# ishine/TargetDiarization

Measured on AMD Instinct MI355X. Metric: real-time factor (audio-sec/wall-sec) full infer() pipe, 16kHz mono, 1/2/4/8 GPU, higher is better.
Workload: dtype f32 (split-f16 x3: fp32-accurate products from three f16 MFMA passes, fp32 accumulate); 1 GPU; BASELINE configs[3]: 1800 s synthetic conversation (two alternating speakers, 20 % overlap) = 180 x 10 s windows: MossFormer2 (90 windows per launch) -> loudness swap -> ERes2NetV2 on every 10 s window of both streams + cosine vs a target embedding -> Paraformer (SANM encoder, CIF predictor, NAR decoder, argmax tokens + timestamps) on 30 s segments of both streams -> CT-Transformer punctuation of ; windows_per_launch=90

## Files before the change

### targetdiarization_amd/csrc/gemm_h3.hpp

```cpp
#pragma once
#include <cstdio>
#include <cstdlib>
#include <typeinfo>
#include <vector>
#include <hip/hip_runtime.h>
#include <stdint.h>

#include "devutil.hpp"
#include "gemm.hpp"

namespace tdx {

typedef _Float16 f16x8 __attribute__((ext_vector_type(8)));

constexpr int H3_BM = 256, H3_BN = 256, H3_BK = 16, H3_THREADS = 512;
constexpr int H3_ROWB = 64;
constexpr int H3_OPER = 256 * H3_ROWB;
constexpr int H3_STAGE = 2 * H3_OPER;
constexpr int H3_NBUF = 4;
constexpr int H3_AUX_AHEAD = 3;
constexpr int H3_LDS = H3_NBUF * H3_STAGE;
constexpr int H3_LDS_EXTRA = 12288;

struct H3Seg {
// ... 725 lines not shown
                    __builtin_amdgcn_sched_barrier(0);
                    if (i + AH < 16) fetch(i + AH, (i + AH) % (AH + 1));
                    const int tn = i >> 3, tm = (i >> 1) & 3, half = i & 1;
                    RowT rw[8];
                    float sr[8];
                    int lb = lrow + tm * 32;
                    asm volatile("" : "+v"(lb));
#pragma unroll
                    for (int r8 = 0; r8 < 8; ++r8) {
                        const int r = half * 8 + r8;
                        const int lr = lb + (r & 3) + 8 * (r >> 2);
                        rw[r8] = row_of(lr);
                        sr[r8] = sal[lr];
                    }
#pragma unroll
                    for (int r8 = 0; r8 < 8; ++r8) touch(ax[i % (AH + 1)][r8]);
                    if (nn[tn] < g.N) {
#pragma unroll
                        for (int r8 = 0; r8 < 8; ++r8) {
                            const int r = half * 8 + r8;
                            const int lr = lb + (r & 3) + 8 * (r >> 2);
                            if constexpr (!CHECK && epi_has_full<Epi>::value) h3_assume_row(rw[r8]);
                            if (!CHECK || m0 + lr < g.M)
                                epi.store(z, m0 + lr, nn[tn], acc[tm][tn][r] * (sr[r8] * sc[tn]), rw[r8], cc[tn], ax[i % (AH + 1)][r8]);
                        }
                    }
                }
            } else {
#pragma unroll
                for (int tn = 0; tn < 2; ++tn) {
                    if (nn[tn] >= g.N) continue;
                    if constexpr (epi_has_ptr<Epi>::value) {
                        float* const p0 = epi.ptr(z, m0 + lrow, nn[tn]);
                        const long ldm = epi.ldm();
                        float sct = sc[tn];
                        if constexpr (epi_has_rowmul<Epi>::value) sct *= epi.colmul(cc[tn]);
#pragma unroll
                        for (int tm = 0; tm < 4; ++tm) {
#pragma unroll
                            for (int r = 0; r < 16; ++r) {
                                const int k = tm * 32 + (r & 3) + 8 * (r >> 2);
                                const RowT rw = row_of(lrow + k);
                                const float sr = sal[lrow + k];
                                if (!CHECK || m0 + lrow + k < g.M) {
                                    if constexpr (epi_has_rowmul<Epi>::value) epi.put_scaled(p0 + k * ldm, acc[tm][tn][r] * (sr * sct), rw, cc[tn]);
                                    else epi.put(p0 + k * ldm, acc[tm][tn][r] * (sr * sct), rw, cc[tn]);
                                }
                            }
                        }
                    } else {
#pragma unroll
                    for (int tm = 0; tm < 4; ++tm) {
#pragma unroll
                        for (int r = 0; r < 16; ++r) {
                            const int lr = lrow + tm * 32 + (r & 3) + 8 * (r >> 2);
                            const RowT rw = row_of(lr);
                            const float sr = sal[lr];
                            if constexpr (!CHECK && epi_has_full<Epi>::value) h3_assume_row(rw);
                            if (!CHECK || m0 + lr < g.M) epi.store(z, m0 + lr, nn[tn], acc[tm][tn][r] * (sr * sc[tn]), rw, cc[tn]);
                        }
                    }
                    }
                }
            }
        }
        }
    };

    auto epilogue_pl = [&](auto tag) {
        if constexpr (epi_has_plout<Epi>::value) {
        constexpr bool CHECK = decltype(tag)::value;
        int lrow = lrow0, lcol = lcol0;
        asm volatile("" : "+v"(lrow), "+v"(lcol));
        float* const T = reinterpret_cast<float*>(lds);
        const H3PlOut po = epi.plout(z);
        auto rowm = [&](int lr) { return CHECK ? min(m0 + lr, g.M - 1) : m0 + lr; };
        __syncthreads();
        if constexpr (PAIRED) {
            static_assert(epi_has_aux<Epi>::value && epi_has_pairmul<Epi>::value, "PLOUT PAIRED: gate-style functor");
            const int c = n0 + lcol;
            auto cc = epi.col(z, c);
            float sc0 = sb[(long)c * sbm], sc1 = sb[(long)(g.pair_off + c) * sbm];
            touch(cc); touch(sc0); touch(sc1);
            { const float2 pm = epi.pairmul(cc); sc0 *= pm.x; sc1 *= pm.y; }
            constexpr int AH = H3_AUX_AHEAD;
            decltype(epi.aux(0, 0, 0, RowT{})) ax[AH + 1][8];
            auto fetch = [&](int hb) {
                int lb = lrow + (hb >> 1) * 32;
                asm volatile("" : "+v"(lb));
#pragma unroll
                for (int r8 = 0; r8 < 8; ++r8) {
                    const int r = (hb & 1) * 8 + r8;
                    const int lr = lb + (r & 3) + 8 * (r >> 2);
                    ax[hb % (AH + 1)][r8] = epi.aux(z, rowm(lr), c, row_of(lr));
                }
            };
#pragma unroll
            for (int hb = 0; hb < AH; ++hb) fetch(hb);
#pragma unroll
            for (int hb = 0; hb < 8; ++hb) {
                __builtin_amdgcn_sched_barrier(0);
                if (hb + AH < 8) fetch(hb + AH);
                RowT rw[8];
                float sr[8];
                int lb = lrow + (hb >> 1) * 32;
                asm volatile("" : "+v"(lb));
#pragma unroll
                for (int r8 = 0; r8 < 8; ++r8) {
                    const int r = (hb & 1) * 8 + r8;
                    const int lr = lb + (r & 3) + 8 * (r >> 2);
                    rw[r8] = row_of(lr);
                    sr[r8] = sal[lr];
                }
#pragma unroll
                for (int r8 = 0; r8 < 8; ++r8) touch(ax[hb % (AH + 1)][r8]);
#pragma unroll
                for (int r8 = 0; r8 < 8; ++r8) {
                    const int tm = hb >> 1, r = (hb & 1) * 8 + r8;
                    const int lr = lb + (r & 3) + 8 * (r >> 2);
                    float v = epi.val2_scaled(z, m0 + lr, c, acc[tm][0][r] * (sr[r8] * sc0), acc[tm][1][r] * (sr[r8] * sc1), rw[r8], cc, ax[hb % (AH + 1)][r8]);
                    if (CHECK && m0 + lr >= g.M) v = 0.f;
                    T[lr * 128 + (lcol ^ (((lr >> 2) & 1) << 5))] = v;
                }
            }
            __syncthreads();
            H3_STAMP(3);
            const int hw = lane >> 5, l32 = lane & 31;
            unsigned char* const pbase = po.planes + (long)n0 * 4;
#pragma unroll 4
            for (int it = 0; it < 16; ++it) {
                const int rl = wave * 32 + it * 2 + hw;
                const int m = m0 + rl;
                const long pr = (!CHECK || m < g.M) ? epi.prow(z, min(m, g.M - 1)) : -1L;
                const f32x4 v4 = *reinterpret_cast<const f32x4*>(T + rl * 128 + ((4 * l32) ^ (((rl >> 2) & 1) << 5)));
                const float4 v = make_float4(v4[0], v4[1], v4[2], v4[3]);
                const float mu = h3_half_max(h3_absmax4(v));
                const float q2 = h3_half_sum((v.x * v.x + v.y * v.y) + (v.z * v.z + v.w * v.w));
                float inv;
                const float sc = h3_row_scale(mu, inv);
                h3_emit4_pred(pbase + (pr < 0 ? 0 : pr) * po.pitch, l32, v, sc, pr >= 0);
                if (l32 == 0 && pr >= 0) {
                    po.scale[(long)bn * po.seg_stride + pr] = inv;
                    if (po.ss) po.ss[(long)bn * po.seg_stride + pr] = q2;
                }
            }
        } else {
            int nn[2];
            decltype(epi.col(0, 0)) cc[2];
            float sc[2];
#pragma unroll
            for (int tn = 0; tn < 2; ++tn) {
                nn[tn] = n0 + tn * 128 + lcol;
                cc[tn] = epi.col(z, nn[tn]);
                sc[tn] = sb[(long)nn[tn] * sbm];
            }
            touch(cc[0]); touch(cc[1]); touch(sc[0]); touch(sc[1]);
            unsigned char* const pbase = po.planes + (long)n0 * 4;
            auto phase2 = [&](int hf) {
                __syncthreads();
#pragma unroll 4
                for (int it = 0; it < 16; ++it) {
                    const int rl = wave * 16 + it;
                    const int lr = (rl >> 6) * 128 + (2 * hf + ((rl >> 5) & 1)) * 32 + (rl & 31);
                    const int m = m0 + lr;
                    const long pr = (!CHECK || m < g.M) ? epi.prow(z, min(m, g.M - 1)) : -1L;
                    const f32x4 v4 = *reinterpret_cast<const f32x4*>(T + rl * 256 + ((4 * lane) ^ (((rl >> 2) & 1) << 5)));
                    const float4 v = make_float4(v4[0], v4[1], v4[2], v4[3]);
                    const float mu = h3_wave_max(h3_absmax4(v));
                    float q2 = (v.x * v.x + v.y * v.y) + (v.z * v.z + v.w * v.w);
                    if (po.ss) q2 = h3_wave_sum(q2);
                    float inv;
                    const float s_ = h3_row_scale(mu, inv);
                    if (pr >= 0) {
                        h3_emit4(pbase + pr * po.pitch, lane, v, s_);
                        if constexpr (epi_has_rowout<Epi>::value) *reinterpret_cast<f32x4*>(epi.rowout(z, pr, n0) + 4 * lane) = v4;
                        if (lane == 0) {
                            po.scale[(long)bn * po.seg_stride + pr] = inv;
                            if (po.ss) po.ss[(long)bn * po.seg_stride + pr] = q2;
                        }
                    }
                }
            };
            if constexpr (epi_has_aux<Epi>::value) {
                constexpr int AH = H3_AUX_AHEAD;
                decltype(epi.aux(0, 0, 0, RowT{})) ax[AH + 1][8];
                auto fetch = [&](int i, int set) {
                    const int tn = (i >> 2) & 1, tm = 2 * (i >> 3) + ((i >> 1) & 1), half = i & 1;
                    int lb = lrow + tm * 32;
                    asm volatile("" : "+v"(lb));
#pragma unroll
                    for (int r8 = 0; r8 < 8; ++r8) {
                        const int r = half * 8 + r8;
                        const int lr = lb + (r & 3) + 8 * (r >> 2);
                        ax[set][r8] = epi.aux(z, rowm(lr), nn[tn], row_of(lr));
                    }
                };
#pragma unroll
                for (int i = 0; i < AH; ++i) fetch(i, i % (AH + 1));
#pragma unroll
                for (int i = 0; i < 16; ++i) {
                    __builtin_amdgcn_sched_barrier(0);
                    if (i == 8) __syncthreads();
                    if (i + AH < 16) fetch(i + AH, (i + AH) % (AH + 1));
                    const int tn = (i >> 2) & 1, tmh = (i >> 1) & 1, tm = 2 * (i >> 3) + tmh, half = i & 1;
                    RowT rw[8];
                    float sr[8];
                    int lb = lrow + tm * 32;
                    asm volatile("" : "+v"(lb));
#pragma unroll
                    for (int r8 = 0; r8 < 8; ++r8) {
                        const int r = half * 8 + r8;
                        const int lr = lb + (r & 3) + 8 * (r >> 2);
                        rw[r8] = row_of(lr);
                        sr[r8] = sal[lr];
                    }
#pragma unroll
                    for (int r8 = 0; r8 < 8; ++r8) touch(ax[i % (AH + 1)][r8]);
#pragma unroll
                    for (int r8 = 0; r8 < 8; ++r8) {
                        const int r = half * 8 + r8;
                        const int lr = lb + (r & 3) + 8 * (r >> 2);
                        float v = 0.f;
                        if (!CHECK || m0 + lr < g.M) v = epi.val(z, m0 + lr, nn[tn], acc[tm][tn][r] * (sr[r8] * sc[tn]), rw[r8], cc[tn], ax[i % (AH + 1)][r8]);
                        const int rl = lr - wm * 64 - (tm - tmh) * 32;
                        T[rl * 256 + ((tn * 128 + lcol) ^ (((rl >> 2) & 1) << 5))] = v;
                    }
                    if (i == 7 || i == 15) phase2(i >> 3);
                }
            } else {
#pragma unroll
                for (int hf = 0; hf < 2; ++hf) {
                    if (hf) __syncthreads();
#pragma unroll
                    for (int tn = 0; tn < 2; ++tn) {
#pragma unroll
                        for (int tmh = 0; tmh < 2; ++tmh) {
                            const int tm = 2 * hf + tmh;
#pragma unroll
                            for (int r = 0; r < 16; ++r) {
                                const int lr = lrow + tm * 32 + (r & 3) + 8 * (r >> 2);
                                const RowT rw = row_of(lr);
                                const float sr = sal[lr];
                                float v = 0.f;
                                if (!CHECK || m0 + lr < g.M) v = epi.val(z, m0 + lr, nn[tn], acc[tm][tn][r] * (sr * sc[tn]), rw, cc[tn]);
                                const int rl = lr - wm * 64 - hf * 64 + 0 * tmh;
                                T[rl * 256 + ((tn * 128 + lcol) ^ (((rl >> 2) & 1) << 5))] = v;
                            }
                        }
                    }
                    phase2(hf);
                }
            }
        }
        }
    };

    auto epilogue_conv = [&]() {
        if constexpr (CONV) {
        int lrow = lrow0, lcol = lcol0;
        asm volatile("" : "+v"(lrow), "+v"(lcol));
        const H3Conv cv = epi.conv();
        int nn[2];
        decltype(epi.col(0, 0)) cc[2];
        float sc[2];
#pragma unroll
        for (int tn = 0; tn < 2; ++tn) {
            nn[tn] = n0 + tn * 128 + lcol;
            const int nc = min(nn[tn], g.N - 1);
            cc[tn] = epi.col(z, nc);
            sc[tn] = sb[(long)nc * sbm] * epi.colmul(cc[tn]);
        }
        touch(cc[0]); touch(cc[1]); touch(sc[0]); touch(sc[1]);
        if (n0 >= cv.ncols) {
#pragma unroll
            for (int tn = 0; tn < 2; ++tn) {
                if (nn[tn] >= g.N) continue;
                float* const p0 = epi.ptr(z, m0 + lrow, nn[tn]);
                const long ldm = epi.ldm();
#pragma unroll
                for (int tm = 0; tm < 4; ++tm) {
#pragma unroll
                    for (int r = 0; r < 16; ++r) {
                        const int k = tm * 32 + (r & 3) + 8 * (r >> 2);
                        const int lr = lrow + k;
                        const RowT rw = row_of(lr);
                        const float sr = sal[lr];
                        if (lr >= H3_CONV_HALO && lr < H3_CONV_HALO + H3_CONV_STEP && m0 + lr < g.M)
                            epi.put_scaled(p0 + k * ldm, acc[tm][tn][r] * (sr * sc[tn]), rw, cc[tn]);
                    }
                }
            }
            return;
        }
        float* const T = reinterpret_cast<float*>(lds);
        int* const sid = reinterpret_cast<int*>(lds + H3_LDS + 4096);
        const bool fast = m0 >= 0 && m0 + 255 < g.M && (m0 / cv.S) == ((m0 + 255) / cv.S);
        if (!fast && tid < 256) { const int m = m0 + tid; sid[tid] = (m >= 0 && m < g.M) ? m / cv.S : -1; }
        typedef float v2f __attribute__((ext_vector_type(2)));
        constexpr int KT = 17, HALF = 8, RW = 30;
        const int r_first = H3_CONV_HALO + RW * wave;
        __syncthreads();
        auto half = [&](auto tnc) {
            constexpr int tn = decltype(tnc)::value;
#pragma unroll
            for (int tm = 0; tm < 4; ++tm) {
#pragma unroll
                for (int j = 0; j < 4; ++j) {
                    const int lr = lrow + tm * 32 + 8 * j;
                    const f32x4 sr4 = *reinterpret_cast<const f32x4*>(sal + lr);
#pragma unroll
                    for (int i = 0; i < 4; ++i) T[(lr + i) * 128 + lcol] = (g.dbg & 16) ? acc[tm][tn][4 * j + i] : epi.act(acc[tm][tn][4 * j + i] * (sr4[i] * sc[tn]), cc[tn]);
                }
            }
            const int colp = n0 + tn * 128 + 2 * lane;
            v2f w[KT];
#pragma unroll
            for (int t = 0; t < KT; ++t) w[t] = *reinterpret_cast<const v2f*>(cv.w + (long)t * cv.wld + colp);
            __syncthreads();
            H3_STAMP(tn == 0 ? 3 : 6);
            const float* const Tc = T + 2 * lane;
            const unsigned poff = (unsigned)((colp >> 5) * 128 + (colp & 31) * 2);
            const bool has32 = cv.u32 && colp >= cv.u0;
            const unsigned uoff = (unsigned)(colp - cv.u0) * 4u;
            auto emit = [&](v2f o, long prow, long m) {
                typedef _Float16 h2 __attribute__((ext_vector_type(2)));
                const v2f xs = o * v2f{cv.sv, cv.sv};
                const h2 hi = h2{(_Float16)xs[0], (_Float16)xs[1]};
                const h2 lo = h2{(_Float16)(xs[0] - (float)hi[0]), (_Float16)(xs[1] - (float)hi[1])};
                unsigned char* const rowp = cv.planes + prow * cv.pitch;
                if (g.dbg & 4) { if (xs[0] == 123.456f) *reinterpret_cast<h2*>(rowp + poff) = lo; return; }
                *reinterpret_cast<h2*>(rowp + poff) = hi;
                *reinterpret_cast<h2*>(rowp + 64 + poff) = lo;
                if (has32) *reinterpret_cast<v2f*>(reinterpret_cast<unsigned char*>(cv.u32 + m * cv.ld32) + uoff) = o;
            };
            if (fast) {
                const int b0 = m0 / cv.S;
                const long prow0 = (long)b0 * cv.Sp + (m0 - b0 * cv.S);
                constexpr int RUN = 10;
#pragma unroll 1
                for (int r0 = r_first; r0 < r_first + RW; r0 += RUN) {
                    v2f win[RUN + KT - 1];
#pragma unroll
                    for (int i = 0; i < RUN + KT - 1; ++i) win[i] = *reinterpret_cast<const v2f*>(Tc + (r0 - HALF + i) * 128);
#pragma unroll
                    for (int i = 0; i < RUN; ++i) {
                        v2f o = win[HALF + i];
                        if (!(g.dbg & 8)) {
#pragma unroll
                            for (int t = 0; t < KT; ++t) o = __builtin_elementwise_fma(w[t], win[i + t], o);
                        }
                        emit(o, prow0 + r0 + i, (long)m0 + r0 + i);
                    }
                }
            } else {
#pragma unroll 1
                for (int lr = r_first; lr < r_first + RW; ++lr) {
                    const int so = sid[lr];
                    if (so < 0) continue;
                    v2f o = *reinterpret_cast<const v2f*>(Tc + lr * 128);
#pragma unroll
                    for (int t = 0; t < KT; ++t) {
                        const int rt = lr + t - HALF;
                        if (sid[rt] == so) o = __builtin_elementwise_fma(w[t], *reinterpret_cast<const v2f*>(Tc + rt * 128), o);
                    }
                    const long m = (long)m0 + lr;
                    emit(o, (long)so * cv.Sp + (m - (long)so * cv.S), m);
                }
            }
        };
        if (g.dbg & 32) return;
        half(std::integral_constant<int, 0>{});
        H3_STAMP(5);
        __syncthreads();
        half(std::integral_constant<int, 1>{});
        }
    };
    if constexpr (CONV) { epilogue_conv(); H3_STAMP(4); return; }
    bool whole = m0 + 256 <= g.M;
    if constexpr (epi_has_full<Epi>::value) whole = whole && epi.full(z, m0);
    if constexpr (epi_has_plout<Epi>::value) { if (whole) epilogue_pl(std::false_type{}); else epilogue_pl(std::true_type{}); }
    else { if (whole) epilogue(std::false_type{}); else epilogue(std::true_type{}); }
    H3_STAMP(4);
}

template <bool A_TR, bool B_TR, bool PAIRED, bool TWOSEG, class Epi, int VARIANT = 0, bool A_CONV = false>
inline hipError_t launch_gemm_h3x(H3Args g, int batches, Epi epi, hipStream_t st) {
    static const hipError_t attr_rc = hipFuncSetAttribute(reinterpret_cast<const void*>(&gemm_h3_kernel<A_TR, B_TR, PAIRED, TWOSEG, Epi, VARIANT, A_CONV>), hipFuncAttributeMaxDynamicSharedMemorySize,
                            H3_LDS + H3_LDS_EXTRA);
    (void)attr_rc;
    g.tiles_m = (g.M + H3_BM - 1) / H3_BM;
    if constexpr (epi_has_conv<Epi>::value) {
        g.tiles_m = (g.M + H3_CONV_STEP - 1) / H3_CONV_STEP;
        if (batches != 1 || g.seg[0].segk || g.seg[0].kchunk) return hipErrorInvalidValue;
    }
    g.tiles_n = PAIRED ? g.N / (H3_BN / 2) : (g.N + H3_BN - 1) / H3_BN;
    g.batches = batches;
    dim3 grid;
    if (g.tiles_m >= 16 && batches <= 4) {
        g.map_mode = 0;
        g.mp = (g.tiles_m + 7) / 8;
        long ktot = 0;
        for (int i = 0; i < g.nseg; ++i) ktot += g.seg[i].K;
        static const long gw_kb = [] { const char* e = getenv("TDX_H3_GW_KB"); return e ? atol(e) : 1536L; }();
        long gw = (gw_kb * 1024) / (256L * ktot * 4);
        if (gw < 1) gw = 1;
        if (gw > g.tiles_n) gw = g.tiles_n;
        g.gw = (int)gw;
        static const int mc_env = [] { const char* e = getenv("TDX_H3_MC"); return e ? atoi(e) : -1; }();
        g.mc = 0;
        if (g.gw < g.tiles_n) {
            long mc = mc_env >= 0 ? mc_env : (6L * 1024 * 1024) / (256L * ktot * 4);
            if (mc > 0 && mc < g.mp) g.mc = (int)mc;
        }
        grid = dim3(8 * g.mp * g.tiles_n, batches, 1);
    } else {
        g.map_mode = 1;
        g.mp = 0; g.gw = 1;
        grid = dim3(8 * ((batches + 7) / 8) * g.tiles_m * g.tiles_n, 1, 1);
    }
    if (TWOSEG && (g.seg[0].K < 64 || g.seg[1].K < 64 || g.seg[0].kchunk || g.seg[1].kchunk)) return hipErrorInvalidValue;
    for (int i = 0; i < g.nseg; ++i) {
        const H3Seg& sg = g.seg[i];
        if (sg.segk && (TWOSEG || A_TR || A_CONV || sg.segk % 64 || sg.K % sg.segk || sg.K / sg.segk > 8 || sg.kchunk)) return hipErrorInvalidValue;
        if ((sg.a_shift || sg.a_period) && (A_TR || A_CONV || (sg.a_period && !sg.a_zero))) return hipErrorInvalidValue;
    }
    if (epi_has_plout<Epi>::value && !PAIRED && g.N % 256) return hipErrorInvalidValue;
    if (A_CONV && (g.cv_cin < 64 || g.cv_cin % 16 || g.seg[0].K != g.cv_ntaps * g.cv_cin || !g.zero_row ||
                   batches != (g.cv_taps_total ? g.cv_taps_total / g.cv_ntaps : 1) || (g.cv_taps_total && g.cv_taps_total % g.cv_ntaps))) return hipErrorInvalidValue;
    static const int dbg = [] { const char* e = getenv("TDX_H3_DEBUG"); return e ? atoi(e) : 0; }();
    g.dbg = dbg;
#ifdef TDX_H3_STAMPS
    static int stamp_calls = 0;
    const long nblk = (long)grid.x * grid.y;
    if (!g.stamps && getenv("TDX_H3_STAMPS_DIR") && nblk >= 512 && ++stamp_calls == 4) {
        unsigned long long* buf = nullptr;
        hipMalloc((void**)&buf, nblk * 64);
        hipMemsetAsync(buf, 0, nblk * 64, st);
        g.stamps = buf;
        g.tiles_n = g.tiles_n;
        hipLaunchKernelGGL((gemm_h3_kernel<A_TR, B_TR, PAIRED, TWOSEG, Epi, VARIANT, A_CONV>), grid, dim3(H3_THREADS), H3_LDS + H3_LDS_EXTRA, st, g, epi);
        hipStreamSynchronize(st);
        std::vector<unsigned long long> hbuf(nblk * 8);
        hipMemcpy(hbuf.data(), buf, nblk * 64, hipMemcpyDeviceToHost);
        long ktot = 0;
        for (int i = 0; i < g.nseg; ++i) ktot += g.seg[i].K;
        char fn[512];
        snprintf(fn, sizeof fn, "%s/h3_%s_M%d_N%d_K%ld_z%d.bin", getenv("TDX_H3_STAMPS_DIR"), typeid(Epi).name(), g.M, g.N, ktot, batches);
        if (FILE* f = fopen(fn, "wb")) { fwrite(hbuf.data(), 8, hbuf.size(), f); fclose(f); }
        hipFree(buf);
        return hipGetLastError();
    }
#endif
    hipLaunchKernelGGL((gemm_h3_kernel<A_TR, B_TR, PAIRED, TWOSEG, Epi, VARIANT, A_CONV>), grid, dim3(H3_THREADS), H3_LDS + H3_LDS_EXTRA, st, g, epi);
    return hipGetLastError();
}

template <bool PAIRED, class Epi, int VARIANT = 0>
inline hipError_t launch_gemm_h3(H3Args g, int batches, Epi epi, hipStream_t st) {
    return launch_gemm_h3x<false, false, PAIRED, false, Epi, VARIANT>(g, batches, epi, st);
}


template <int UNUSED = 0>
__global__ __launch_bounds__(256) void h3_split_rows_kernel(const float* __restrict__ x, long ld, unsigned char* __restrict__ planes,
                                                           float* __restrict__ scale, long R, int K, int Kp) {
    const int lane = threadIdx.x & 63;
    const long row = (long)blockIdx.x * 4 + (threadIdx.x >> 6);
    if (row >= R) return;
    const float* xr = x + row * ld;
    float v[4][8];
    float mu = 0.f;
    const int nch = Kp / 8;
#pragma unroll
    for (int c = 0; c < 4; ++c) {
        const int ch = lane + 64 * c;
#pragma unroll
        for (int i = 0; i < 8; ++i) v[c][i] = 0.f;
        if (ch * 8 < K) {
            const f32x4 a = ldg4(xr + ch * 8), b = ldg4(xr + ch * 8 + 4);
#pragma unroll
            for (int i = 0; i < 4; ++i) { v[c][i] = a[i]; v[c][4 + i] = b[i]; }
        }
#pragma unroll
        for (int i = 0; i < 8; ++i) mu = fmaxf(mu, fabsf(v[c][i]));
    }
#pragma unroll
    for (int o = 32; o >= 1; o >>= 1) mu = fmaxf(mu, __shfl_xor(mu, o, 64));
    float inv;
    const float s = h3_row_scale(mu, inv);
    unsigned char* pr = planes + row * (long)Kp * 4;
#pragma unroll
    for (int c = 0; c < 4; ++c) {
        const int ch = lane + 64 * c;
        if (ch < nch) h3_store_chunk(pr + ch * 32, v[c], s);
    }
    if (lane == 0) scale[row] = inv;
}

template <int UNUSED = 0>
__global__ __launch_bounds__(256) void h3_split_rows_static_kernel(const float* __restrict__ x, long ld, unsigned char* __restrict__ planes,
                                                                  long R, int K, int Kp, float s) {
    const long i = (long)blockIdx.x * 256 + threadIdx.x;
    const int per = Kp / 8;
    if (i >= R * per) return;
    const long row = i / per;
    const int ch = (int)(i - row * per);
    float v[8];
#pragma unroll
    for (int j = 0; j < 8; ++j) v[j] = 0.f;
    if (ch * 8 < K) {
        const f32x4 a = ldg4(x + row * ld + ch * 8), b = ldg4(x + row * ld + ch * 8 + 4);
#pragma unroll
        for (int j = 0; j < 4; ++j) { v[j] = a[j]; v[4 + j] = b[j]; }
    }
    h3_store_chunk(planes + row * (long)Kp * 4 + ch * 32, v, s);
}
inline hipError_t launch_h3_split_rows_static(const float* x, long ld, void* planes, long R, int K, float s, hipStream_t st) {
    const int Kp = (K + 15) / 16 * 16;
    const long n = R * (Kp / 8);
    hipLaunchKernelGGL(h3_split_rows_static_kernel<0>, dim3((unsigned)((n + 255) / 256)), dim3(256), 0, st, x, ld, (unsigned char*)planes, R, K, Kp, s);
    return hipGetLastError();
}

template <int UNUSED = 0>
__global__ __launch_bounds__(256) void h3_split_rows_long_kernel(const float* __restrict__ x, long ld, unsigned char* __restrict__ planes,
                                                                float* __restrict__ scale, int K) {
    __shared__ float wmax[4];
    const long row = blockIdx.x;
    const float* xr = x + row * ld;
    float mu = 0.f;
    for (int k = threadIdx.x * 4; k < K; k += 1024) mu = fmaxf(mu, h3_absmax4(*reinterpret_cast<const float4*>(xr + k)));
    mu = h3_wave_max(mu);
    if ((threadIdx.x & 63) == 0) wmax[threadIdx.x >> 6] = mu;
    __syncthreads();
    mu = fmaxf(fmaxf(wmax[0], wmax[1]), fmaxf(wmax[2], wmax[3]));
    float inv;
    const float s = h3_row_scale(mu, inv);
    for (int ch = threadIdx.x; ch < K / 8; ch += 256) {
        const f32x4 a = ldg4(xr + ch * 8), b = ldg4(xr + ch * 8 + 4);
        const float v[8] = {a[0], a[1], a[2], a[3], b[0], b[1], b[2], b[3]};
        h3_store_chunk(planes + row * (long)K * 4 + ch * 32, v, s);
    }
    if (threadIdx.x == 0) scale[row] = inv;
}
inline hipError_t launch_h3_split_rows_long(const float* x, long ld, void* planes, float* scale, long R, int K, hipStream_t st) {
    hipLaunchKernelGGL(h3_split_rows_long_kernel<0>, dim3((unsigned)R), dim3(256), 0, st, x, ld, (unsigned char*)planes, scale, K);
    return hipGetLastError();
}

template <int UNUSED = 0>
__global__ __launch_bounds__(256) void h3_split_kmajor_kernel(const float* __restrict__ x, long ld, unsigned char* __restrict__ planes,
                                                             long K, int N, float s, const unsigned* __restrict__ mx,
                                                             float* __restrict__ inv, int S, int Sp) {
    const long i = (long)blockIdx.x * 256 + threadIdx.x;
    const int per = N / 8;
    if (i >= K * per) return;
    const long k = i / per;
    const int n = (int)(i - k * per) * 8;
    if (mx) {
        float iv;
        s = h3_row_scale(__uint_as_float(mx[0]), iv);
        if (i == 0) inv[0] = iv;
    }
    long src = k;
    bool ok = true;
    if (Sp > 0) { const long b = k / Sp; const int t = (int)(k - b * Sp); ok = t < S; src = b * S + t; }
    f32x4 a = {0.f, 0.f, 0.f, 0.f}, b4 = {0.f, 0.f, 0.f, 0.f};
    if (ok) { a = ldg4(x + src * ld + n); b4 = ldg4(x + src * ld + n + 4); }
    const float v[8] = {a[0], a[1], a[2], a[3], b4[0], b4[1], b4[2], b4[3]};
    f16x8 hi, lo;
#pragma unroll
    for (int j = 0; j < 8; ++j) {
        const float xs = v[j] * s;
        const _Float16 t = (_Float16)xs;
        hi[j] = t; lo[j] = (_Float16)(xs - (float)t);
    }
    unsigned char* dst = planes + k * (4L * N) + (n >> 5) * 128 + ((n & 31) >> 3) * 16;
    *reinterpret_cast<f16x8*>(dst) = hi;
    *reinterpret_cast<f16x8*>(dst + 64) = lo;
}

template <int UNUSED = 0>
__global__ __launch_bounds__(256) void h3_absmax_kernel(const float* __restrict__ x, long n, unsigned* __restrict__ mx) {
    float m = 0.f;
    for (long i = (long)blockIdx.x * 256 + threadIdx.x; i < n; i += (long)gridDim.x * 256) m = fmaxf(m, fabsf(x[i]));
    m = h3_wave_max(m);
    if ((threadIdx.x & 63) == 0) atomicMax(mx, __float_as_uint(m));
}

inline hipError_t launch_h3_split_rows(const float* x, long ld, void* planes, float* scale, long R, int K, hipStream_t st) {
    const int Kp = (K + 15) / 16 * 16;
    hipLaunchKernelGGL(h3_split_rows_kernel<0>, dim3((unsigned)((R + 3) / 4)), dim3(256), 0, st, x, ld, (unsigned char*)planes, scale, R, K, Kp);
    return hipGetLastError();
}

}
```

Baseline: 512.0 audio-s/s.

## Widen conv epilogue stores via lane permutes and swizzled LDS staging

Reworks the fused depthwise-conv epilogue of the split-f16 GEMM. Each lane now owns a column permutation, and staged tiles in LDS use an XOR-swizzled column layout. Two adjacent output rows are exchanged across lanes with permlane32/permlane16 swaps, so hi/lo f16 plane writes and fp32 side-output writes become 16-byte stores instead of scattered 4/8-byte stores. The FMA loop is reordered tap-outer to expose independent accumulators. In exchange it adds permute instructions and register pressure, and it depends on the has32 region starting at the tile column base, a coarser check than the previous per-column one.

After: 514.9 audio-s/s, median of 6. Within noise of the previous version (+0.6%).

```diff
diff --git a/targetdiarization_amd/csrc/gemm_h3.hpp b/targetdiarization_amd/csrc/gemm_h3.hpp
--- a/targetdiarization_amd/csrc/gemm_h3.hpp
+++ b/targetdiarization_amd/csrc/gemm_h3.hpp
@@ -1051,54 +1051,81 @@
         __syncthreads();
         auto half = [&](auto tnc) {
             constexpr int tn = decltype(tnc)::value;
-#pragma unroll
-            for (int tm = 0; tm < 4; ++tm) {
-#pragma unroll
-                for (int j = 0; j < 4; ++j) {
-                    const int lr = lrow + tm * 32 + 8 * j;
-                    const f32x4 sr4 = *reinterpret_cast<const f32x4*>(sal + lr);
-#pragma unroll
-                    for (int i = 0; i < 4; ++i) T[(lr + i) * 128 + lcol] = (g.dbg & 16) ? acc[tm][tn][4 * j + i] : epi.act(acc[tm][tn][4 * j + i] * (sr4[i] * sc[tn]), cc[tn]);
-                }
-            }
-            const int colp = n0 + tn * 128 + 2 * lane;
+            const int pcol = 32 * ((lcol >> 1) & 3) + ((((lcol >> 2) & ~1) | (lcol & 1)) ^ (8 * ((lcol >> 1) & 3)));
+            auto stage = [&](auto actc) {
+#pragma unroll
+                for (int tm = 0; tm < 4; ++tm) {
+#pragma unroll
+                    for (int j = 0; j < 4; ++j) {
+                        const int lr = lrow + tm * 32 + 8 * j;
+                        const f32x4 sr4 = *reinterpret_cast<const f32x4*>(sal + lr);
+#pragma unroll
+                        for (int i = 0; i < 4; ++i)
+                            T[(lr + i) * 128 + pcol] = decltype(actc)::value ? epi.act(acc[tm][tn][4 * j + i] * (sr4[i] * sc[tn]), cc[tn]) : acc[tm][tn][4 * j + i];
+                    }
+                }
+            };
+            if (g.dbg & 16) stage(std::false_type{});
+            else stage(std::true_type{});
+            const int colbase = n0 + tn * 128;
+            const int colp = colbase + 8 * (lane & 15) + 2 * (lane >> 4);
             v2f w[KT];
 #pragma unroll
             for (int t = 0; t < KT; ++t) w[t] = *reinterpret_cast<const v2f*>(cv.w + (long)t * cv.wld + colp);
             __syncthreads();
             H3_STAMP(tn == 0 ? 3 : 6);
-            const float* const Tc = T + 2 * lane;
-            const unsigned poff = (unsigned)((colp >> 5) * 128 + (colp & 31) * 2);
-            const bool has32 = cv.u32 && colp >= cv.u0;
-            const unsigned uoff = (unsigned)(colp - cv.u0) * 4u;
-            auto emit = [&](v2f o, long prow, long m) {
-                typedef _Float16 h2 __attribute__((ext_vector_type(2)));
+            const float* const Tc = T + 32 * (lane >> 4) + ((2 * (lane & 15)) ^ (8 * (lane >> 4)));
+            const bool has32 = cv.u32 && colbase >= cv.u0;
+            typedef _Float16 h2 __attribute__((ext_vector_type(2)));
+            auto split = [&](v2f o, unsigned& hiw, unsigned& low) {
                 const v2f xs = o * v2f{cv.sv, cv.sv};
                 const h2 hi = h2{(_Float16)xs[0], (_Float16)xs[1]};
                 const h2 lo = h2{(_Float16)(xs[0] - (float)hi[0]), (_Float16)(xs[1] - (float)hi[1])};
-                unsigned char* const rowp = cv.planes + prow * cv.pitch;
-                if (g.dbg & 4) { if (xs[0] == 123.456f) *reinterpret_cast<h2*>(rowp + poff) = lo; return; }
-                *reinterpret_cast<h2*>(rowp + poff) = hi;
-                *reinterpret_cast<h2*>(rowp + 64 + poff) = lo;
-                if (has32) *reinterpret_cast<v2f*>(reinterpret_cast<unsigned char*>(cv.u32 + m * cv.ld32) + uoff) = o;
+                hiw = __builtin_bit_cast(unsigned, hi); low = __builtin_bit_cast(unsigned, lo);
             };
             if (fast) {
                 const int b0 = m0 / cv.S;
                 const long prow0 = (long)b0 * cv.Sp + (m0 - b0 * cv.S);
+                const int t4 = lane >> 4, b16 = lane & 15;
+                const unsigned pofs = (unsigned)(colbase * 4 + (b16 >> 2) * 128 + (t4 & 1) * 64 + (b16 & 3) * 16 + (t4 >> 1) * cv.pitch);
+                const unsigned uofs = (unsigned)(((colbase - cv.u0) + 8 * b16 + 4 * (t4 & 1)) * 4 + (t4 >> 1) * cv.ld32 * 4);
+                auto swap32 = [](unsigned& x, unsigned& y) { const auto r = __builtin_amdgcn_permlane32_swap(x, y, false, false); x = r[0]; y = r[1]; };
+                auto swap16 = [](unsigned& x, unsigned& y) { const auto r = __builtin_amdgcn_permlane16_swap(x, y, false, false); x = r[0]; y = r[1]; };
                 constexpr int RUN = 10;
 #pragma unroll 1
                 for (int r0 = r_first; r0 < r_first + RW; r0 += RUN) {
                     v2f win[RUN + KT - 1];
 #pragma unroll
                     for (int i = 0; i < RUN + KT - 1; ++i) win[i] = *reinterpret_cast<const v2f*>(Tc + (r0 - HALF + i) * 128);
-#pragma unroll
-                    for (int i = 0; i < RUN; ++i) {
-                        v2f o = win[HALF + i];
-                        if (!(g.dbg & 8)) {
-#pragma unroll
-                            for (int t = 0; t < KT; ++t) o = __builtin_elementwise_fma(w[t], win[i + t], o);
+                    v2f o[RUN];
+#pragma unroll
+                    for (int i = 0; i < RUN; ++i) o[i] = win[HALF + i];
+                    if (!(g.dbg & 8)) {
+#pragma unroll
+                        for (int t = 0; t < KT; ++t)
+#pragma unroll
+                            for (int i = 0; i < RUN; ++i) o[i] = __builtin_elementwise_fma(w[t], win[i + t], o[i]);
+                    }
+                    unsigned char* const rowp = cv.planes + (prow0 + r0) * cv.pitch;
+                    unsigned char* const urow = reinterpret_cast<unsigned char*>(cv.u32 + ((long)m0 + r0) * cv.ld32);
+                    if (g.dbg & 4) {
+                        if (o[0][0] == 123.456f && o[RUN - 1][1] == 123.456f) *reinterpret_cast<v2f*>(rowp) = o[0];
+                        continue;
+                    }
+#pragma unroll
+                    for (int p = 0; p < RUN; p += 2) {
+                        unsigned x0, x1, x2, x3;
+                        split(o[p], x0, x1); split(o[p + 1], x2, x3);
+                        swap32(x0, x2); swap32(x1, x3); swap16(x0, x1); swap16(x2, x3);
+                        *reinterpret_cast<uint4*>(rowp + (long)p * cv.pitch + pofs) = make_uint4(x0, x1, x2, x3);
+                    }
+                    if (has32) {
+#pragma unroll
+                        for (int p = 0; p < RUN; p += 2) {
+                            unsigned u0 = __float_as_uint(o[p][0]), u1 = __float_as_uint(o[p][1]), u2 = __float_as_uint(o[p + 1][0]), u3 = __float_as_uint(o[p + 1][1]);
+                            swap32(u0, u2); swap32(u1, u3); swap16(u0, u2); swap16(u1, u3);
+                            *reinterpret_cast<uint4*>(urow + (long)p * cv.ld32 * 4 + uofs) = make_uint4(u0, u1, u2, u3);
                         }
-                        emit(o, prow0 + r0 + i, (long)m0 + r0 + i);
                     }
                 }
             } else {
@@ -1113,7 +1140,14 @@
                         if (sid[rt] == so) o = __builtin_elementwise_fma(w[t], *reinterpret_cast<const v2f*>(Tc + rt * 128), o);
                     }
                     const long m = (long)m0 + lr;
-                    emit(o, (long)so * cv.Sp + (m - (long)so * cv.S), m);
+                    unsigned hiw, low;
+                    split(o, hiw, low);
+                    unsigned char* const rowp = cv.planes + ((long)so * cv.Sp + (m - (long)so * cv.S)) * cv.pitch;
+                    const unsigned poff = (unsigned)((colp >> 5) * 128 + (colp & 31) * 2);
+                    if (g.dbg & 4) { if (o[0] == 123.456f) *reinterpret_cast<unsigned*>(rowp + poff) = low; continue; }
+                    *reinterpret_cast<unsigned*>(rowp + poff) = hiw;
+                    *reinterpret_cast<unsigned*>(rowp + 64 + poff) = low;
+                    if (has32) *reinterpret_cast<v2f*>(reinterpret_cast<unsigned char*>(cv.u32 + m * cv.ld32) + (unsigned)(colp - cv.u0) * 4u) = o;
                 }
             }
         };
```
